# rapidsai/wholegraph

Measured on AMD Instinct MI355X. Metric: gather_GBps_out (gathered output row bytes/s, reference gather_scatter_bench convention), higher is better.
Workload: dtype f32

## Files before the change

include/wholememory/wholegraph_amd_ext.h:

```cpp
#ifndef WHOLEMEMORY_WHOLEGRAPH_AMD_EXT_H_
#define WHOLEMEMORY_WHOLEGRAPH_AMD_EXT_H_

#include <wholememory/embedding.h>
#include <wholememory/wholememory_op.h>

#ifdef __cplusplus
extern "C" {
#endif

struct wm_ext_collectives_t {
  void* ctx;
  int (*barrier)(void* ctx);
  int (*allgather_host)(void* ctx, const void* send, void* recv, size_t bytes);
  int (*alltoallv_device)(void* ctx,
                          const void* send,
                          const size_t* send_bytes,
                          const size_t* send_disp,
                          void* recv,
                          const size_t* recv_bytes,
                          const size_t* recv_disp,
                          void* stream);
};
#ifndef __cplusplus
typedef struct wm_ext_collectives_t wm_ext_collectives_t;
// ... 62 lines not shown
wholememory_error_code_t wholememory_ext_sample_append_unique(
  wholememory_tensor_t wm_csr_row_ptr_tensor, wholememory_tensor_t wm_csr_col_ptr_tensor,
  wholememory_tensor_t center_nodes_tensor, int max_sample_count, unsigned long long random_seed,
  wholememory_tensor_t output_sample_offset_tensor, void* output_unique_memory_context,
  void* output_neighbor_pos_memory_context, void* output_center_localid_memory_context, wholememory_env_func_t* p_env_fns,
  void* stream);

wholememory_error_code_t wholememory_ext_weighted_sample_append_unique(
  wholememory_tensor_t wm_csr_row_ptr_tensor, wholememory_tensor_t wm_csr_col_ptr_tensor,
  wholememory_tensor_t wm_csr_weight_ptr_tensor, wholememory_tensor_t center_nodes_tensor, int max_sample_count,
  unsigned long long random_seed, wholememory_tensor_t output_sample_offset_tensor, void* output_unique_memory_context,
  void* output_neighbor_pos_memory_context, void* output_center_localid_memory_context, wholememory_env_func_t* p_env_fns,
  void* stream);

enum wholememory_error_code_t wholememory_ext_multilayer_sample(
  wholememory_tensor_t wm_csr_row_ptr_tensor, wholememory_tensor_t wm_csr_col_ptr_tensor, wholememory_tensor_t seed_nodes_tensor,
  int hops, const int* max_sample_counts, const unsigned long long* random_seeds, void* const* sample_offsets,
  void* const* unique, int* const* neighbor_pos, int* const* center_lid, int* counts_host,
  struct wholememory_env_func_t* p_env_fns, void* stream);

enum wholememory_error_code_t wholememory_ext_multilayer_sample_weighted(
  wholememory_tensor_t wm_csr_row_ptr_tensor, wholememory_tensor_t wm_csr_col_ptr_tensor,
  wholememory_tensor_t wm_csr_weight_ptr_tensor, wholememory_tensor_t seed_nodes_tensor, int hops, const int* max_sample_counts,
  const unsigned long long* random_seeds, void* const* sample_offsets, void* const* unique, int* const* neighbor_pos,
  int* const* center_lid, int* counts_host, struct wholememory_env_func_t* p_env_fns, void* stream);

enum wholememory_error_code_t wholememory_ext_sample_append_unique_edges(
  wholememory_tensor_t wm_csr_row_ptr_tensor, wholememory_tensor_t wm_csr_col_ptr_tensor,
  wholememory_tensor_t wm_csr_weight_ptr_tensor, wholememory_tensor_t center_nodes_tensor, int max_sample_count,
  unsigned long long random_seed, wholememory_tensor_t output_sample_offset_tensor, void* output_unique_memory_context,
  void* output_neighbor_pos_memory_context, void* output_center_localid_memory_context, void* output_edge_gid_memory_context,
  struct wholememory_env_func_t* p_env_fns, void* stream);

enum wholememory_error_code_t wholememory_ext_multilayer_sample_edges(
  wholememory_tensor_t wm_csr_row_ptr_tensor, wholememory_tensor_t wm_csr_col_ptr_tensor,
  wholememory_tensor_t wm_csr_weight_ptr_tensor, wholememory_tensor_t seed_nodes_tensor, int hops, const int* max_sample_counts,
  const unsigned long long* random_seeds, void* const* sample_offsets, void* const* unique, int* const* neighbor_pos,
  int* const* center_lid, int64_t* const* edge_gid, int n_attrs, const wholememory_tensor_t* attr_tensors,
  void* const* attr_out, int* counts_host, struct wholememory_env_func_t* p_env_fns, void* stream);

int64_t wholememory_ext_edge_chain_calls(void);

enum wholememory_error_code_t wholememory_ext_set_async_completion(int on);

enum wholememory_error_code_t wholememory_ext_reload_knobs(void);

enum wholememory_error_code_t wholememory_ext_probe_memory(void* ptr, size_t bytes, int kind, int reps, float* ms_per_gib);

enum wholememory_error_code_t wholememory_ext_set_malloc_probe(const char* mode);
enum wholememory_error_code_t wholememory_ext_get_malloc_probe(char* mode, size_t capacity);
int wholememory_ext_handle_was_probed(wholememory_handle_t handle);

int64_t wholememory_ext_host_sorted_gathers(void);

int64_t wholememory_ext_split_sorts(void);

void wholememory_ext_agg_grid_stats(int64_t* launches, int64_t* truncated);

int64_t wholememory_ext_dense_fold_last(void);

int64_t wholememory_ext_distributed_gather_launches(void);

int64_t wholememory_ext_distributed_scatter_launches(void);

int64_t wholememory_ext_gradient_exchange_launches(void);

int64_t wholememory_ext_alltoallv_bytes(void);

int64_t wholememory_ext_combined_gradient_calls(void);

enum wholememory_ext_aggr_t {
  WHOLEMEMORY_EXT_AGGR_SUM  = 0,
  WHOLEMEMORY_EXT_AGGR_MEAN = 1,
};
enum wholememory_error_code_t wholememory_ext_csc_aggregate_forward(const int32_t* row_ptr,
                                                                    const int32_t* col_ind,
                                                                    int64_t n_edges,
                                                                    int64_t n_dst,
                                                                    int64_t n_src,
                                                                    const float* x,
                                                                    int64_t x_stride,
                                                                    int64_t dim,
                                                                    int aggr,
                                                                    float* out,
                                                                    int64_t out_stride,
                                                                    struct wholememory_env_func_t* p_env_fns,
                                                                    void* stream);
enum wholememory_error_code_t wholememory_ext_csc_aggregate_backward(const int32_t* row_ptr,
                                                                     const int32_t* col_ind,
                                                                     int64_t n_edges,
                                                                     int64_t n_dst,
                                                                     int64_t n_src,
                                                                     const float* grad_out,
                                                                     int64_t grad_out_stride,
                                                                     int64_t dim,
                                                                     int aggr,
                                                                     float* grad_x,
                                                                     int64_t grad_x_stride,
                                                                     struct wholememory_env_func_t* p_env_fns,
                                                                     void* stream);
int64_t wholememory_ext_csc_aggregate_chunk_edges(void);

enum wholememory_error_code_t wholememory_ext_csc_aggregate_forward_typed(const int32_t* row_ptr,
                                                                          const int32_t* col_ind,
                                                                          int64_t n_edges,
                                                                          int64_t n_dst,
// ... 450 lines not shown
```

wholegraph_amd/binding.py:

```python
import ctypes as C
import os

_HERE = os.path.dirname(os.path.abspath(__file__))
LIB_PATH = os.path.join(_HERE, "libwholegraph.so")

WHOLEMEMORY_SUCCESS = 0
NOT_SUPPORTED = 9
OUT_OF_MEMORY = 8
ERROR_NAMES = {
    0: "WHOLEMEMORY_SUCCESS", 1: "WHOLEMEMORY_UNKNOW_ERROR", 2: "WHOLEMEMORY_NOT_IMPLEMENTED",
    3: "WHOLEMEMORY_LOGIC_ERROR", 4: "WHOLEMEMORY_CUDA_ERROR", 5: "WHOLEMEMORY_COMMUNICATION_ERROR",
    6: "WHOLEMEMORY_INVALID_INPUT", 7: "WHOLEMEMORY_INVALID_VALUE", 8: "WHOLEMEMORY_OUT_OF_MEMORY",
    9: "WHOLEMEMORY_NOT_SUPPORTED", 10: "WHOLEMEMORY_SYSTEM_ERROR",
}
MT_NONE, MT_CONTINUOUS, MT_CHUNKED, MT_DISTRIBUTED, MT_HIERARCHY = range(5)
ML_NONE, ML_DEVICE, ML_HOST = range(3)
(DT_UNKNOWN, DT_FLOAT, DT_HALF, DT_DOUBLE, DT_BF16, DT_INT, DT_INT64, DT_INT16, DT_INT8, DT_COUNT) = range(10)
MA_NONE, MA_DEVICE, MA_HOST, MA_PINNED = range(4)
AGGR_SUM, AGGR_MEAN = range(2)
PNA_AGGR = {"sum": 1, "mean": 2, "min": 4, "max": 8, "std": 16}
OPT_NONE, OPT_SGD, OPT_LAZY_ADAM, OPT_RMSPROP, OPT_ADAGRAD = range(5)
AT_NONE, AT_READONLY, AT_READWRITE = range(3)
LEVEL_FATAL, LEVEL_ERROR, LEVEL_WARN, LEVEL_INFO, LEVEL_DEBUG, LEVEL_TRACE = range(6)
MAX_TENSOR_DIM = 8
# ... 161 lines not shown
    "wholememory_tensor_get_entry_partition_sizes": (_i, [_P(_sz), _vp]),
    "wholememory_tensor_get_local_entry_count": (_i, [_P(_sz), _vp]),
    "wholememory_tensor_get_local_entry_start": (_i, [_P(_sz), _vp]),
    "wholememory_tensor_get_subtensor": (_i, [_vp, _P(_i64), _P(_i64), _P(_vp)]),
    "wholememory_tensor_get_root": (_vp, [_vp]),
    "get_wholememory_tensor_count": (_i64, []),
    "get_device_prop": (_vp, [_i]),
    "wholememory_get_default_env_func": (_P(EnvFunc), []),
    "wholememory_get_cached_env_func": (_P(EnvFunc), []),
    "wholememory_drop_cached_env_func_cache": (None, []),
    "wholememory_gather": (_i, [_vp, _vp, _vp, _P(EnvFunc), _vp, _i]),
    "wholememory_scatter": (_i, [_vp, _vp, _vp, _P(EnvFunc), _vp, _i]),
    "wholememory_create_embedding_optimizer": (_i, [_P(_vp), _i]),
    "wholememory_optimizer_set_parameter": (_i, [_vp, C.c_char_p, _vp]),
    "wholememory_destroy_embedding_optimizer": (None, [_vp]),
    "wholememory_create_embedding_cache_policy": (_i, [_P(_vp), _vp, _i, _i, _i, _f]),
    "wholememory_destroy_embedding_cache_policy": (_i, [_vp]),
    "wholememory_create_embedding": (_i, [_P(_vp), _P(TensorDescription), _vp, _i, _i, _vp, _P(_sz), _i, _i]),
    "wholememory_destroy_embedding": (_i, [_vp]),
    "wholememory_embedding_get_embedding_tensor": (_vp, [_vp]),
    "wholememory_embedding_set_optimizer": (_i, [_vp, _vp]),
    "wholememory_embedding_gather": (_i, [_vp, _vp, _vp, _b, _P(EnvFunc), _i64]),
    "wholememory_embedding_gather_gradient_apply": (_i, [_vp, _vp, _vp, _b, _f, _P(EnvFunc), _i64]),
    "wholememory_embedding_get_optimizer_state_names": (_P(C.c_char_p), [_vp]),
    "wholememory_embedding_get_optimizer_state": (_vp, [_vp, C.c_char_p]),
    "wholememory_embedding_writeback_cache": (_i, [_vp, _i64]),
    "wholememory_embedding_drop_all_cache": (_i, [_vp, _i64]),
    "wholememory_env_test_op": (_i, [_vp, _vp, _vp, _vp, _vp, _i64, _P(EnvFunc), _vp]),
    "wholegraph_csr_unweighted_sample_without_replacement": (_i, [_vp, _vp, _vp, _i, _vp, _vp, _vp, _vp, C.c_ulonglong,
                                                                 _P(EnvFunc), _vp]),
    "wholegraph_csr_weighted_sample_without_replacement": (_i, [_vp, _vp, _vp, _vp, _i, _vp, _vp, _vp, _vp,
                                                               C.c_ulonglong, _P(EnvFunc), _vp]),
    "generate_random_positive_int_cpu": (_i, [_i64, _i64, _vp]),
    "generate_exponential_distribution_negative_float_cpu": (_i, [_i64, _i64, _vp]),
    "graph_append_unique": (_i, [_vp, _vp, _vp, _vp, _P(EnvFunc), _vp]),
    "csr_add_self_loop": (_i, [_vp, _vp, _vp, _vp, _vp]),
    "wholememory_create_communicator_ext": (_i, [_P(_vp), _i, _i, _P(ExtCollectives)]),
    "wholememory_ext_communicator_transport": (_i, [_vp, _P(C.c_char_p), _P(_i)]),
    "wholememory_ext_bucket_ids": (_i, [_vp, _i, _i64, _vp, _i, _vp, _vp, _vp, _P(EnvFunc), _vp]),
    "wholememory_ext_bucket_ids_folded": (_i, [_vp, _i, _i64, _vp, _i, _i, _vp, _vp, _vp, _P(EnvFunc), _vp]),
    "wholememory_ext_dedup_apply": (_i, [_vp, _i, _i64, _vp, _i64, _i64, _vp, _i64, _i64, _i64, _i, _P(_f), _f, _vp,
                                        _vp, _P(_i64), _P(EnvFunc), _vp]),
    "wholememory_ext_round_robin_map": (_i, [_vp, _vp, _i, _i64, _i64, _i, _i, _vp]),
    "wholememory_ext_embedding_cache_info": (_i, [_vp, _P(_i64), _P(_i64), _P(_i64), _P(_i64), _P(_i64)]),
    "wholememory_ext_backend_name": (C.c_char_p, []),
    "wholememory_ext_last_rows_kernel": (C.c_char_p, []),
    "wholememory_ext_sample_append_unique": (C.c_int, [C.c_void_p, C.c_void_p, C.c_void_p, C.c_int, C.c_ulonglong, C.c_void_p,
                                                      C.c_void_p, C.c_void_p, C.c_void_p, C.c_void_p, C.c_void_p]),
    "wholememory_ext_weighted_sample_append_unique": (_i, [_vp, _vp, _vp, _vp, _i, C.c_ulonglong, _vp, _vp, _vp, _vp, _vp, _vp]),
    "wholememory_ext_set_async_completion": (_i, [_i]),
    "wholememory_ext_reload_knobs": (_i, []),
    "wholememory_ext_probe_memory": (_i, [_vp, C.c_size_t, _i, _i, _P(_f)]),
    "wholememory_ext_host_sorted_gathers": (_i64, []),
    "wholememory_ext_split_sorts": (_i64, []),
    "wholememory_ext_agg_grid_stats": (None, [_P(_i64), _P(_i64)]),
    "wholememory_ext_dense_fold_last": (_i64, []),
    "wholememory_ext_distributed_gather_launches": (_i64, []),
    "wholememory_ext_distributed_scatter_launches": (_i64, []),
    "wholememory_ext_gradient_exchange_launches": (_i64, []),
    "wholememory_ext_alltoallv_bytes": (_i64, []),
    "wholememory_ext_combined_gradient_calls": (_i64, []),
    "wholememory_ext_set_malloc_probe": (_i, [C.c_char_p]),
    "wholememory_ext_get_malloc_probe": (_i, [C.c_char_p, C.c_size_t]),
    "wholememory_ext_handle_was_probed": (_i, [_vp]),
    "wholememory_ext_multilayer_sample": (_i, [_vp, _vp, _vp, _i, _vp, _vp, _vp, _vp, _vp, _vp, _vp, _vp, _vp]),
    "wholememory_ext_multilayer_sample_weighted": (_i, [_vp, _vp, _vp, _vp, _i, _vp, _vp, _vp, _vp, _vp, _vp, _vp, _vp, _vp]),
    "wholememory_ext_sample_append_unique_edges": (_i, [_vp, _vp, _vp, _vp, _i, C.c_ulonglong, _vp, _vp, _vp, _vp, _vp, _vp, _vp]),
    "wholememory_ext_multilayer_sample_edges": (_i, [_vp, _vp, _vp, _vp, _i, _vp, _vp, _vp, _vp, _vp, _vp, _vp, _i, _vp, _vp, _vp,
                                                    _vp, _vp]),
    "wholememory_ext_edge_chain_calls": (_i64, []),
    "wholememory_ext_csr_random_walk": (_i, [_vp, _vp, _vp, _vp, _i, C.c_ulonglong, _vp, _vp, _vp]),
    "wholememory_ext_csr_node2vec_walk": (_i, [_vp, _vp, _vp, _vp, _i, C.c_float, C.c_float, _i, C.c_ulonglong, _vp, _vp, _vp]),
    "wholememory_ext_csr_negative_sample": (_i, [_vp, _vp, _vp, _i, _i, _i, _i, _i, C.c_ulonglong, _vp, _vp]),
    "wholememory_ext_csr_induced_subgraph": (_i, [_vp, _vp, _vp, _vp, _vp, _vp, _P(EnvFunc), _vp]),
    "wholememory_ext_csc_aggregate_forward": (_i, [_vp, _vp, _i64, _i64, _i64, _vp, _i64, _i64, _i, _vp, _i64, _P(EnvFunc),
                                                  _vp]),
    "wholememory_ext_csc_aggregate_backward": (_i, [_vp, _vp, _i64, _i64, _i64, _vp, _i64, _i64, _i, _vp, _i64, _P(EnvFunc),
                                                   _vp]),
    "wholememory_ext_csc_aggregate_chunk_edges": (_i64, []),
    "wholememory_ext_csc_aggregate_forward_typed": (_i, [_vp, _vp, _i64, _i64, _i64, _vp, _i64, _i64, _i, _vp, _i64, _i,
                                                        _P(EnvFunc), _vp]),
    "wholememory_ext_csc_aggregate_backward_typed": (_i, [_vp, _vp, _i64, _i64, _i64, _vp, _i64, _i64, _i, _vp, _i64, _i,
                                                         _P(EnvFunc), _vp]),
    "wholememory_ext_csc_aggregate_weighted_forward": (_i, [_vp, _vp, _vp, _i64, _i64, _i64, _vp, _i64, _i64, _i, _vp, _i64,
                                                           _P(EnvFunc), _vp]),
    "wholememory_ext_csc_gather_aggregate_forward": (_i, [_vp, _vp, _i, _vp, _vp, _i64, _i64, _i64, _i, _vp, _i64, _P(EnvFunc),
                                                         _vp]),
    "wholememory_ext_gather_aggregate_calls": (_i64, []),
    "wholememory_ext_csc_aggregate_weighted_backward": (_i, [_vp, _vp, _i64, _i64, _i64, _vp, _i64, _vp, _vp, _i64, _i64, _i,
                                                            _vp, _i64, _vp, _P(EnvFunc), _vp]),
    "wholememory_ext_csc_gat_forward": (_i, [_vp, _vp, _i64, _i64, _i64, _vp, _i64, _vp, _i64, _i64, C.c_float, _i, _vp,
                                            _i64, _vp, _vp, _P(EnvFunc), _vp]),
    "wholememory_ext_csc_gat_backward": (_i, [_vp, _vp, _i64, _i64, _i64, _vp, _i64, _vp, _i64, _i64, C.c_float, _i, _vp,
                                             _vp, _vp, _i64, _vp, _i64, _vp, _P(EnvFunc), _vp]),
    "wholememory_ext_csc_gat_node_chunk": (_i64, []),
    "wholememory_ext_csc_gat_edge_forward": (_i, [_vp, _vp, _i64, _i64, _i64, _vp, _i64, _vp, _vp, _i64, _i64, _i64,
                                                 C.c_float, _i, _vp, _i64, _vp, _vp, _vp, _P(EnvFunc), _vp]),
    "wholememory_ext_csc_gat_edge_backward": (_i, [_vp, _vp, _i64, _i64, _i64, _vp, _i64, _vp, _vp, _i64, _i64, _i64,
                                                  C.c_float, _i, _vp, _vp, _vp, _vp, _i64, _vp, _i64, _vp, _vp, _i64,
                                                  _P(EnvFunc), _vp]),
    "wholememory_ext_csc_gatv2_forward": (_i, [_vp, _vp, _i64, _i64, _i64, _vp, _i64, _vp, _i64, _vp, _i64, _i64,
                                              C.c_float, _i, _vp, _i64, _vp, _P(EnvFunc), _vp]),
    "wholememory_ext_csc_gatv2_backward": (_i, [_vp, _vp, _i64, _i64, _i64, _vp, _i64, _vp, _i64, _vp, _i64, _i64,
                                               C.c_float, _i, _vp, _vp, _i64, _vp, _i64, _vp, _i64, _vp, _P(EnvFunc),
                                               _vp]),
    "wholememory_ext_csc_mha_simple_forward": (_i, [_vp, _vp, _i64, _i64, _i64, _vp, _i64, _vp, _i64, _vp, _i64, _i64, _i64,
# ... 72 lines not shown
```

wholegraph_amd/csrc/embedding_cache.cpp:

```cpp
#include "embedding_cache.hpp"

#include <algorithm>
#include <cstring>

namespace wm {

row_cache::~row_cache()
{
  const auto* bk = backend();
  if (args.slot_of) bk->free_device(args.slot_of);
  if (args.count) bk->free_device(args.count);
  if (args.row_of) bk->free_device(args.row_of);
  if (args.dirty) bk->free_device(args.dirty);
  if (args.data) bk->free_device(args.data);
  if (args.data2) bk->free_device(args.data2);
  if (counters_dev) bk->free_device(counters_dev);
}

wholememory_error_code_t create_row_cache(row_cache** out, const wholememory_embedding_cache_policy_* policy,
                                          wholememory_tensor_t raw, wholememory_comm_t embedding_comm)
{
  const auto* bk = backend();
  if (bk->cache_update == nullptr) return WHOLEMEMORY_NOT_SUPPORTED;
  auto* desc = wholememory_tensor_get_tensor_description(raw);
  auto h     = wholememory_tensor_get_memory_handle(raw);
  std::unique_ptr<row_cache> c(new row_cache());
  c->same_comm = policy->cache_comm == embedding_comm;
  c->writable  = policy->access_type == WHOLEMEMORY_AT_READWRITE;
  c->dtype     = desc->dtype;
  c->row_elems = desc->strides[0];
  c->raw       = raw;
  const size_t es = wholememory_dtype_get_element_size(desc->dtype);
  auto& a         = c->args;
  a.row_bytes     = c->row_elems * static_cast<int64_t>(es);
  if (a.row_bytes % 16 != 0) return WHOLEMEMORY_LOGIC_ERROR;
  a.raw_row_stride_bytes = a.row_bytes;
  a.raw_row_offset_bytes = desc->storage_offset * static_cast<int64_t>(es);
  if (c->same_comm) {
    std::vector<size_t> off = entry_offsets_of(h, static_cast<size_t>(a.row_bytes));
    a.cover_start           = static_cast<int64_t>(off[embedding_comm->world_rank]);
    a.cover_rows            = static_cast<int64_t>(off[embedding_comm->world_rank + 1]) - a.cover_start;
    a.raw_gref              = local_shard_gref(h);
  } else {
    a.cover_start = 0;
    a.cover_rows  = desc->sizes[0];
    if (wholememory_get_memory_type(h) == WHOLEMEMORY_MT_DISTRIBUTED && embedding_comm->world_size > 1) {
      c->raw_addressable = false;
      a.raw_gref         = wholememory_create_continuous_global_reference(nullptr);
    } else {
      WHOLEMEMORY_RETURN_ON_FAIL(tensor_mapped_gref(raw, &a.raw_gref));
    }
  }
  if (a.cover_rows >= (INT64_C(1) << 31)) return WHOLEMEMORY_NOT_SUPPORTED;
  int64_t slots = static_cast<int64_t>(static_cast<double>(a.cover_rows) * policy->cache_ratio);
  slots         = std::min(a.cover_rows + 63, std::max<int64_t>(slots, a.cover_rows > 0 ? 64 : 0));
  a.n_sets      = (slots + 63) / 64;
  a.set_cover   = a.n_sets > 0 ? (a.cover_rows + a.n_sets - 1) / a.n_sets : 0;
  const int64_t n_slots = a.n_sets * 64;
  auto dev_alloc = [&](void** p, size_t bytes) { WM_BK(bk->malloc_device(p, std::max<size_t>(bytes, 16))); };
  dev_alloc(reinterpret_cast<void**>(&a.slot_of), sizeof(int32_t) * a.cover_rows);
  dev_alloc(reinterpret_cast<void**>(&a.count), sizeof(int32_t) * a.cover_rows);
  dev_alloc(reinterpret_cast<void**>(&a.row_of), sizeof(int64_t) * n_slots);
  dev_alloc(reinterpret_cast<void**>(&a.dirty), n_slots);
  dev_alloc(reinterpret_cast<void**>(&a.data), static_cast<size_t>(n_slots) * a.row_bytes);
  dev_alloc(reinterpret_cast<void**>(&c->counters_dev), 32);
  WM_BK(bk->memset_async(a.slot_of, 0xff, sizeof(int32_t) * a.cover_rows, nullptr));
  WM_BK(bk->memset_async(a.count, 0, sizeof(int32_t) * a.cover_rows, nullptr));
  WM_BK(bk->memset_async(a.row_of, 0xff, sizeof(int64_t) * n_slots, nullptr));
  WM_BK(bk->memset_async(a.dirty, 0, n_slots, nullptr));
  WM_BK(bk->memset_async(c->counters_dev, 0, 32, nullptr));
  WM_BK(bk->stream_sync(nullptr));
  *out = c.release();
  return WHOLEMEMORY_SUCCESS;
}

wholememory_error_code_t row_cache_update(row_cache* c, const void* ids, wholememory_dtype_t index_dtype, int64_t n,
                                          int64_t key_upper_bound, wholememory_env_func_t* env, void* stream)
{
  const auto* bk = backend();
  if (n == 0 || c->args.n_sets == 0) return WHOLEMEMORY_SUCCESS;
  if (n >= (INT64_C(1) << 31)) return WHOLEMEMORY_INVALID_INPUT;
  sorted_ids s(env);
  int rc = s.run(ids, index_dtype, n, key_upper_bound, 0, stream);
  if (rc != 0) return rc == -1 ? WHOLEMEMORY_INVALID_INPUT : WHOLEMEMORY_CUDA_ERROR;
  rc = bk->cache_update(&c->args, s.unique, index_dtype, s.starts, s.n_unique_dev, n, nullptr, nullptr, nullptr, stream);
  if (rc != 0) return rc == -1 ? WHOLEMEMORY_INVALID_INPUT : WHOLEMEMORY_CUDA_ERROR;
  WM_BK(bk->stream_sync(stream));
  return WHOLEMEMORY_SUCCESS;
}

wholememory_error_code_t row_cache_plan(row_cache* c, const void* ids, wholememory_dtype_t index_dtype, int64_t n, int64_t key_upper_bound,
                                        wholememory_env_func_t* env, void* stream, temp_mem* rows_mem, temp_mem* slots_mem,
                                        int64_t* n_fill)
{
  const auto* bk = backend();
  *n_fill        = 0;
  auto* fill_rows  = static_cast<int64_t*>(rows_mem->device(n, WHOLEMEMORY_DT_INT64));
  auto* fill_slots = static_cast<int64_t*>(slots_mem->device(n, WHOLEMEMORY_DT_INT64));
  if (n == 0 || c->args.n_sets == 0) return WHOLEMEMORY_SUCCESS;
  if (n >= (INT64_C(1) << 31) || c->writable) return WHOLEMEMORY_INVALID_INPUT;
  sorted_ids s(env);
  temp_mem count(env), host_n(env);
  auto* d_count = static_cast<int*>(count.device(1, WHOLEMEMORY_DT_INT));
  WM_BK(bk->memset_async(d_count, 0, sizeof(int), stream));
  int rc = s.run(ids, index_dtype, n, key_upper_bound, 0, stream);
  if (rc != 0) return rc == -1 ? WHOLEMEMORY_INVALID_INPUT : WHOLEMEMORY_CUDA_ERROR;
  rc = bk->cache_update(&c->args, s.unique, index_dtype, s.starts, s.n_unique_dev, n, fill_rows, fill_slots, d_count, stream);
  if (rc != 0) return rc == -1 ? WHOLEMEMORY_INVALID_INPUT : WHOLEMEMORY_CUDA_ERROR;
  auto* h = static_cast<int*>(host_n.pinned(1, WHOLEMEMORY_DT_INT));
  WM_BK(bk->memcpy_async(h, d_count, sizeof(int), stream));
  WM_BK(bk->stream_sync(stream));
  *n_fill = *h;
  return WHOLEMEMORY_SUCCESS;
}

wholememory_error_code_t row_cache_install(row_cache* c, const void* rows_data, const int64_t* slots, int64_t n_fill,
                                           void* stream)
{
  const auto* bk = backend();
  if (n_fill == 0) return WHOLEMEMORY_SUCCESS;
  wm_rows_args a{};
  a.gref          = wholememory_create_continuous_global_reference(c->args.data);
  a.table_dtype   = c->dtype;
  a.dim           = c->row_elems;
  a.table_stride  = c->row_elems;
  a.indices       = slots;
  a.index_dtype   = WHOLEMEMORY_DT_INT64;
  a.n             = n_fill;
  a.plain         = const_cast<void*>(rows_data);
  a.plain_dtype   = c->dtype;
  a.plain_stride  = c->row_elems;
  a.max_blocks    = -1;
  WM_BK(bk->scatter_rows(&a, stream));
  return WHOLEMEMORY_SUCCESS;
}

wholememory_error_code_t row_cache_split(row_cache* c, const void* ids, wholememory_dtype_t index_dtype, int64_t n,
                                         int64_t* cache_idx, void* raw_idx, void* stream)
{
  int rc = backend()->cache_split(&c->args, ids, index_dtype, n, cache_idx, raw_idx, c->counters_dev, stream);
  if (rc != 0) return rc == -1 ? WHOLEMEMORY_INVALID_INPUT : WHOLEMEMORY_CUDA_ERROR;
  c->lookups += n;
  return WHOLEMEMORY_SUCCESS;
}

wholememory_error_code_t row_cache_gather(row_cache* c, const wm_rows_args& a, wholememory_env_func_t* env, void* stream)
{
  const auto* bk = backend();
  if (a.n == 0) return WHOLEMEMORY_SUCCESS;
  temp_mem cache_idx_mem(env), raw_idx_mem(env);
  auto* cache_idx = static_cast<int64_t*>(cache_idx_mem.device(a.n, WHOLEMEMORY_DT_INT64));
  void* raw_idx   = raw_idx_mem.device(a.n, a.index_dtype);
  WHOLEMEMORY_RETURN_ON_FAIL(row_cache_split(c, a.indices, a.index_dtype, a.n, cache_idx, raw_idx, stream));
  wm_rows_args hit        = a;
  hit.gref                = wholememory_create_continuous_global_reference(c->args.data);
  hit.table_stride        = c->row_elems;
  hit.table_storage_offset = 0;
  hit.indices             = cache_idx;
  hit.index_dtype         = WHOLEMEMORY_DT_INT64;
  WM_BK(bk->gather_rows(&hit, stream));
  wm_rows_args miss = a;
  miss.indices      = raw_idx;
  WM_BK(bk->gather_rows(&miss, stream));
  WM_BK(bk->stream_sync(stream));
  return WHOLEMEMORY_SUCCESS;
}

wholememory_error_code_t row_cache_attach_states(row_cache* c, wholememory_tensor_t state_local)
{
  const auto* bk = backend();
  if (!c->same_comm || !c->writable || c->args.data2 != nullptr) return WHOLEMEMORY_INVALID_INPUT;
  WHOLEMEMORY_RETURN_ON_FAIL(row_cache_writeback(c, true, nullptr));
  auto* d = wholememory_tensor_get_tensor_description(state_local);
  if (d->dtype != WHOLEMEMORY_DT_FLOAT || d->dim != 2) return WHOLEMEMORY_INVALID_INPUT;
  auto& a                 = c->args;
  a.row_bytes2            = d->strides[0] * static_cast<int64_t>(sizeof(float));
  a.raw2_row_stride_bytes = a.row_bytes2;
  if (a.row_bytes2 % 16 != 0) return WHOLEMEMORY_LOGIC_ERROR;
  char* local = static_cast<char*>(wholememory_tensor_get_data_pointer(state_local));
  a.raw2_gref = wholememory_create_continuous_global_reference(local - a.cover_start * a.row_bytes2);
  void* p     = nullptr;
  WM_BK(bk->malloc_device(&p, std::max<size_t>(static_cast<size_t>(a.n_sets) * 64 * a.row_bytes2, 16)));
  a.data2 = static_cast<char*>(p);
  return WHOLEMEMORY_SUCCESS;
}

wholememory_error_code_t row_cache_writeback(row_cache* c, bool drop, void* stream)
{
  const auto* bk = backend();
  int rc         = bk->cache_writeback(&c->args, drop ? 1 : 0, stream);
  if (rc != 0) return WHOLEMEMORY_CUDA_ERROR;
  return bk->stream_sync(stream) == 0 ? WHOLEMEMORY_SUCCESS : WHOLEMEMORY_CUDA_ERROR;
}

wholememory_error_code_t row_cache_info(row_cache* c, int64_t* slots, int64_t* occupied, int64_t* dirty, int64_t* hits,
                                        int64_t* lookups, void* stream)
{
  const auto* bk = backend();
  if (bk->cache_info(&c->args, c->counters_dev + 1, stream) != 0) return WHOLEMEMORY_CUDA_ERROR;
  unsigned long long h[3] = {0, 0, 0};
  WM_BK(bk->memcpy_async(h, c->counters_dev, sizeof(h), stream));
  WM_BK(bk->stream_sync(stream));
  if (slots) *slots = c->args.n_sets * 64;
  if (occupied) *occupied = static_cast<int64_t>(h[1]);
  if (dirty) *dirty = static_cast<int64_t>(h[2]);
  if (hits) *hits = static_cast<int64_t>(h[0]);
  if (lookups) *lookups = c->lookups;
  return WHOLEMEMORY_SUCCESS;
}

}
```

wholegraph_amd/csrc/embedding_cache.hpp:

```cpp
#pragma once

#include <wholememory/embedding.h>

#include "backend.hpp"
#include "ops_internal.hpp"

struct wholememory_embedding_cache_policy_ {
  wholememory_comm_t cache_comm;
  wholememory_memory_type_t cache_memory_type;
  wholememory_memory_location_t cache_memory_location;
  wholememory_access_type_t access_type;
  float cache_ratio;
};

namespace wm {

struct row_cache {
  wm_cache_args args{};
  bool same_comm = false;
  bool writable  = false;
  bool raw_addressable = true;
  wholememory_tensor_t raw = nullptr;
  wholememory_dtype_t dtype = WHOLEMEMORY_DT_UNKNOWN;
  int64_t row_elems         = 0;
  unsigned long long* counters_dev = nullptr;
  int64_t lookups                  = 0;
  ~row_cache();
};

wholememory_error_code_t create_row_cache(row_cache** out, const wholememory_embedding_cache_policy_* policy,
                                          wholememory_tensor_t raw, wholememory_comm_t embedding_comm);

wholememory_error_code_t row_cache_update(row_cache* c, const void* ids, wholememory_dtype_t index_dtype, int64_t n,
                                          int64_t key_upper_bound, wholememory_env_func_t* env, void* stream);

wholememory_error_code_t row_cache_gather(row_cache* c, const wm_rows_args& a, wholememory_env_func_t* env, void* stream);

wholememory_error_code_t row_cache_plan(row_cache* c, const void* ids, wholememory_dtype_t index_dtype, int64_t n,
                                        int64_t key_upper_bound, wholememory_env_func_t* env, void* stream, temp_mem* rows_mem, temp_mem* slots_mem,
                                        int64_t* n_fill);
wholememory_error_code_t row_cache_install(row_cache* c, const void* rows_data, const int64_t* slots, int64_t n_fill,
                                           void* stream);
wholememory_error_code_t row_cache_split(row_cache* c, const void* ids, wholememory_dtype_t index_dtype, int64_t n,
                                         int64_t* cache_idx, void* raw_idx, void* stream);

wholememory_error_code_t row_cache_attach_states(row_cache* c, wholememory_tensor_t state_local);

wholememory_error_code_t row_cache_writeback(row_cache* c, bool drop, void* stream);
wholememory_error_code_t row_cache_info(row_cache* c, int64_t* slots, int64_t* occupied, int64_t* dirty, int64_t* hits,
                                        int64_t* lookups, void* stream);

}
```

wholegraph_amd/csrc/kernels/cache.hip:

```cpp
#include <hip/hip_runtime.h>
#include <stdint.h>

#include <algorithm>

#include "../backend.hpp"

namespace wm {
namespace {

constexpr int kBlock = 256;

struct raw_view {
  char* base;
  char* const* rank_ptrs;
  const size_t* rank_offsets;
  size_t chunk_stride;
  int world_size;
  int same_chunk;
  int64_t row_stride_bytes;
  int64_t row_offset_bytes;
};

struct raw2_view {
  char* base;
// ... 29 lines not shown
  size_t start;
  if (v.same_chunk) {
    rank  = static_cast<int>(off / v.chunk_stride);
    start = static_cast<size_t>(rank) * v.chunk_stride;
  } else {
    rank = 0;
    for (int r = 1; r < v.world_size; r++)
      if (off >= v.rank_offsets[r]) rank = r;
    start = v.rank_offsets[rank];
  }
  return v.rank_ptrs[rank] + (off - start);
}

__device__ __forceinline__ void wave_copy_row(char* dst, const char* src, int row_bytes, int lane)
{
  typedef uint32_t u32x4 __attribute__((ext_vector_type(4)));
  for (int o = lane * 16; o < row_bytes; o += 64 * 16) *reinterpret_cast<u32x4*>(dst + o) = *reinterpret_cast<const u32x4*>(src + o);
}

struct cache_dev {
  int32_t* slot_of;
  int32_t* count;
  int64_t* row_of;
  uint8_t* dirty;
  char* data;
  int64_t cover_start, cover_rows, n_sets, set_cover;
  int row_bytes;
  char* data2;
  int row_bytes2;
};

inline cache_dev make_dev(const wm_cache_args& c)
{
  return cache_dev{c.slot_of, c.count, c.row_of, c.dirty, c.data, c.cover_start, c.cover_rows, c.n_sets, c.set_cover,
                   static_cast<int>(c.row_bytes), c.data2, static_cast<int>(c.row_bytes2)};
}

template <typename IdxT>
__global__ void cache_count_kernel(cache_dev c, const IdxT* unique_rows, const int32_t* run_starts, const int64_t* n_unique)
{
  const int64_t u = static_cast<int64_t>(blockIdx.x) * blockDim.x + threadIdx.x;
  if (u >= *n_unique) return;
  const int64_t r = static_cast<int64_t>(unique_rows[u]) - c.cover_start;
  if (r < 0 || r >= c.cover_rows) return;
  c.count[r] += run_starts[u + 1] - run_starts[u];
}

struct fill_list {
  int64_t* rows;
  int64_t* slots;
  int* count;
};

template <typename IdxT>
__global__ __launch_bounds__(kBlock) void cache_update_kernel(cache_dev c, raw_view raw, raw2_view raw2,
                                                              const IdxT* unique_rows, const int64_t* n_unique_p,
                                                              fill_list fill)
{
  const int lane    = threadIdx.x & 63;
  const int64_t set = (static_cast<int64_t>(blockIdx.x) * kBlock + threadIdx.x) >> 6;
  if (set >= c.n_sets) return;
  const int64_t nu  = *n_unique_p;
  const int64_t lo_row = c.cover_start + set * c.set_cover;
  const int64_t hi_row = min(c.cover_start + c.cover_rows, lo_row + c.set_cover);
  auto lower = [&](int64_t key) {
    int64_t a = 0, b = nu;
    while (a < b) {
      const int64_t m = (a + b) >> 1;
      const IdxT v    = unique_rows[m];
      if (v >= 0 && static_cast<int64_t>(v) < key)
        a = m + 1;
      else
        b = m;
    }
    return a;
  };
  const int64_t first = lower(lo_row), last = lower(hi_row);
  if (first >= last) return;
  const int64_t slot  = set * 64 + lane;
  int64_t my_row      = c.row_of[slot];
  int32_t my_cnt      = my_row >= 0 ? c.count[my_row] : -1;
  for (int64_t j = first; j < last; j++) {
    const int64_t g = static_cast<int64_t>(unique_rows[j]);
    const int64_t r = g - c.cover_start;
    if (c.slot_of[r] >= 0) continue;
    const int32_t cand = c.count[r];
    uint64_t key = (static_cast<uint64_t>(static_cast<uint32_t>(my_cnt + 1)) << 8) | static_cast<uint32_t>(lane);
    for (int off = 32; off > 0; off >>= 1) {
      const uint64_t o = __shfl_xor(key, off, 64);
      key              = o < key ? o : key;
    }
    const int victim      = static_cast<int>(key & 0xff);
    const int32_t min_cnt = static_cast<int32_t>(key >> 8) - 1;
    if (cand <= min_cnt) continue;
    const int64_t vslot = set * 64 + victim;
    char* line          = c.data + vslot * c.row_bytes;
    const int64_t old   = __shfl(my_row, victim, 64);
    if (old >= 0) {
      if (fill.rows == nullptr && c.dirty[vslot]) {
        wave_copy_row(raw_row(raw, c.cover_start + old), line, c.row_bytes, lane);
        if (c.data2 != nullptr)
          wave_copy_row(raw2.base + (c.cover_start + old) * raw2.row_stride_bytes, c.data2 + vslot * c.row_bytes2, c.row_bytes2, lane);
      }
      if (lane == 0) c.slot_of[old] = -1;
    }
    if (fill.rows == nullptr) {
      wave_copy_row(line, raw_row(raw, g), c.row_bytes, lane);
      if (c.data2 != nullptr)
        wave_copy_row(c.data2 + vslot * c.row_bytes2, raw2.base + g * raw2.row_stride_bytes, c.row_bytes2, lane);
    } else if (lane == 0) {
      const int k   = atomicAdd(fill.count, 1);
      fill.rows[k]  = g;
      fill.slots[k] = vslot;
    }
    if (lane == 0) {
      c.slot_of[r]    = static_cast<int32_t>(vslot);
      c.row_of[vslot] = r;
      c.dirty[vslot]  = 0;
    }
    if (lane == victim) {
      my_row = r;
      my_cnt = cand;
    }
    __builtin_amdgcn_fence(__ATOMIC_RELEASE, "agent");
  }
}

template <typename IdxT>
__global__ __launch_bounds__(kBlock) void cache_split_kernel(cache_dev c, const IdxT* ids, int64_t n, int64_t* cache_idx,
                                                             IdxT* raw_idx, unsigned long long* hits)
{
  __shared__ unsigned int block_hits;
  if (threadIdx.x == 0) block_hits = 0;
  __syncthreads();
  unsigned int wave_hits = 0;
  for (int64_t base = static_cast<int64_t>(blockIdx.x) * kBlock; base < n; base += static_cast<int64_t>(gridDim.x) * kBlock) {
    const int64_t i = base + threadIdx.x;
    bool hit        = false;
    if (i < n) {
      const IdxT id   = ids[i];
      const int64_t r = static_cast<int64_t>(id) - c.cover_start;
      int32_t slot    = -1;
      if (id >= 0 && r >= 0 && r < c.cover_rows) slot = c.slot_of[r];
      hit          = slot >= 0;
      cache_idx[i] = slot;
      raw_idx[i]   = hit ? static_cast<IdxT>(-1) : id;
    }
    wave_hits += static_cast<unsigned int>(__popcll(__ballot(hit)));
  }
  if (hits != nullptr) {
    if ((threadIdx.x & 63) == 0 && wave_hits) atomicAdd(&block_hits, wave_hits);
    __syncthreads();
    if (threadIdx.x == 0 && block_hits) atomicAdd(hits, static_cast<unsigned long long>(block_hits));
  }
}

__global__ __launch_bounds__(kBlock) void cache_writeback_kernel(cache_dev c, raw_view raw, raw2_view raw2, int drop)
{
  const int lane     = threadIdx.x & 63;
  const int64_t slot = (static_cast<int64_t>(blockIdx.x) * kBlock + threadIdx.x) >> 6;
  if (slot >= c.n_sets * 64) return;
  const int64_t r = c.row_of[slot];
  if (r < 0) return;
  if (c.dirty[slot]) {
    wave_copy_row(raw_row(raw, c.cover_start + r), c.data + slot * c.row_bytes, c.row_bytes, lane);
    if (c.data2 != nullptr)
      wave_copy_row(raw2.base + (c.cover_start + r) * raw2.row_stride_bytes, c.data2 + slot * c.row_bytes2, c.row_bytes2, lane);
  }
  if (lane == 0) {
    c.dirty[slot] = 0;
    if (drop) {
      c.slot_of[r]   = -1;
      c.row_of[slot] = -1;
    }
  }
}

// ... 88 lines not shown
```

wholegraph_amd/csrc/ops.cpp:

```cpp
#include "knobs.hpp"
#include "ops_internal.hpp"
#include "embedding_cache.hpp"

#include <algorithm>
#include <atomic>
#include <cstdlib>
#include <cstring>

namespace wm {

temp_mem::temp_mem(wholememory_env_func_t* env) : env_(env)
{
  WM_CHECK(env != nullptr, "p_env_fns must not be null");
  env_->temporary_fns.create_memory_context_fn(&ctx_, env_->temporary_fns.global_context);
}
temp_mem::~temp_mem()
{
  if (ptr_ != nullptr) env_->temporary_fns.free_fn(ctx_, env_->temporary_fns.global_context);
  env_->temporary_fns.destroy_memory_context_fn(ctx_, env_->temporary_fns.global_context);
}
void* temp_mem::alloc(int64_t elt_count, wholememory_dtype_t dtype, wholememory_memory_allocation_type_t type)
{
  WM_CHECK(ptr_ == nullptr, "temp_mem slot reused");
  wholememory_tensor_description_t d;
// ... 675 lines not shown
  temp_mem fetched(env), relay_rows(env), back_rows(env);
  char* fetched_buf = static_cast<char*>(fetched.device(dim * n_fetch, d.plain.dtype));
  op_descs db       = d;
  db.indices_ptr    = fetch_ids;
  db.indices        = wholememory_create_array_desc(n_fetch, 0, d.indices.dtype);
  db.plain_ptr      = fetched_buf;
  int64_t fsz[2]    = {n_fetch, dim};
  db.plain          = wholememory_create_matrix_desc(fsz, dim, 0, d.plain.dtype);
  WHOLEMEMORY_RETURN_ON_FAIL(gather_distributed_rows(handle, db, env, stream, gather_sms, nullptr, false, &rail));

  char* send_buf = fetched_buf;
  WM_DEBUG("HIERARCHY gather: rank %d (local %d of %d, node %d of %d) asked %ld ids, relays %ld, fetches %ld distinct",
           comm->world_rank, local_comm->world_rank, L, cross_comm->world_rank, X, static_cast<long>(n),
           static_cast<long>(n_relay), static_cast<long>(n_fetch));
  if (dedup) {
    send_buf       = static_cast<char*>(relay_rows.device(dim * n_relay, d.plain.dtype));
    int64_t rsz[2] = {n_relay, dim};
    auto relay_desc = wholememory_create_matrix_desc(rsz, dim, 0, d.plain.dtype);
    wm_rows_args ea{};
    fill_rows_args(&ea, wholememory_create_continuous_global_reference(fetched_buf), db.plain, inv, WHOLEMEMORY_DT_INT64,
                   n_relay, send_buf, relay_desc, gather_sms);
    WM_BK(bk->gather_rows(&ea, stream));
  }

  const size_t row_bytes = static_cast<size_t>(dim) * oes;
  char* back_buf = static_cast<char*>(back_rows.device(dim * xa.total_valid, d.plain.dtype));
  exchange_segments(local_comm, send_buf, xa.recv_counts, xa.recv_offsets, back_buf, xa.send_counts, xa.bucket_offsets,
                    row_bytes, stream);
  if (xa.total_valid > 0) {
    int64_t bsz[2] = {xa.total_valid, dim};
    auto back_desc = wholememory_create_matrix_desc(bsz, dim, 0, d.plain.dtype);
    wm_rows_args ra{};
    fill_rows_args(&ra, wholememory_create_continuous_global_reference(d.plain_ptr), d.plain, xa.raw_indices,
                   WHOLEMEMORY_DT_INT64, xa.total_valid, back_buf, back_desc, -1);
    WM_BK(bk->scatter_rows(&ra, stream));
  }
  WM_BK(bk->stream_sync(stream));
  return WHOLEMEMORY_SUCCESS;
}

}

wholememory_error_code_t gather_cached(wholememory_tensor_t table, wholememory_tensor_t indices_tensor,
                                       wholememory_tensor_t output_tensor, wholememory_env_func_t* env, void* stream,
                                       int gather_sms, row_cache* cache, bool adjust_cache)
{
  op_descs d;
  WHOLEMEMORY_RETURN_ON_FAIL(check_args(table, indices_tensor, output_tensor, "output", &d));
  auto handle = wholememory_tensor_get_memory_handle(table);
  if (cache->same_comm)
    return gather_distributed_rows(handle, d, env, stream, gather_sms, cache, adjust_cache);
  if (cache->raw_addressable) {
    if (adjust_cache)
      WHOLEMEMORY_RETURN_ON_FAIL(row_cache_update(cache, d.indices_ptr, d.indices.dtype, d.indices.size, d.table.sizes[0], env, stream));
    wm_rows_args a{};
    fill_rows_args(&a, cache->args.raw_gref, d.table, d.indices_ptr, d.indices.dtype, d.indices.size, d.plain_ptr, d.plain,
                   gather_sms);
    return row_cache_gather(cache, a, env, stream);
  }
  const auto* bk     = backend();
  const int64_t n    = d.indices.size;
  const int64_t dim  = d.table.sizes[1];
  if (adjust_cache) {
    temp_mem rows_mem(env), slots_mem(env), staging(env);
    int64_t n_fill = 0;
    WHOLEMEMORY_RETURN_ON_FAIL(row_cache_plan(cache, d.indices_ptr, d.indices.dtype, n, d.table.sizes[0], env, stream, &rows_mem, &slots_mem, &n_fill));
    char* rows_data = static_cast<char*>(staging.device(n_fill * cache->row_elems, d.table.dtype));
    op_descs df     = d;
    df.indices_ptr  = rows_mem.get();
    df.indices      = wholememory_create_array_desc(n_fill, 0, WHOLEMEMORY_DT_INT64);
    df.plain_ptr    = rows_data;
    int64_t fsz[2]  = {n_fill, dim};
    df.plain        = wholememory_create_matrix_desc(fsz, cache->row_elems, 0, d.table.dtype);
    WHOLEMEMORY_RETURN_ON_FAIL(gather_distributed_rows(handle, df, env, stream, gather_sms));
    WHOLEMEMORY_RETURN_ON_FAIL(row_cache_install(cache, rows_data, static_cast<const int64_t*>(slots_mem.get()), n_fill, stream));
    WM_BK(bk->stream_sync(stream));
  }
  temp_mem cache_idx_mem(env), raw_idx_mem(env);
  auto* cache_idx = static_cast<int64_t*>(cache_idx_mem.device(n, WHOLEMEMORY_DT_INT64));
  void* raw_idx   = raw_idx_mem.device(n, d.indices.dtype);
  WHOLEMEMORY_RETURN_ON_FAIL(row_cache_split(cache, d.indices_ptr, d.indices.dtype, n, cache_idx, raw_idx, stream));
  if (n > 0) {
    wm_rows_args hit{};
    fill_rows_args(&hit, wholememory_create_continuous_global_reference(cache->args.data), d.table, cache_idx,
                   WHOLEMEMORY_DT_INT64, n, d.plain_ptr, d.plain, gather_sms);
    hit.table_stride         = cache->row_elems;
    hit.table_storage_offset = 0;
    WM_BK(bk->gather_rows(&hit, stream));
  }
  op_descs dm    = d;
  dm.indices_ptr = raw_idx;
  dm.indices.storage_offset = 0;
  WHOLEMEMORY_RETURN_ON_FAIL(gather_distributed(handle, dm, env, stream, gather_sms));
  WM_BK(bk->stream_sync(stream));
  return WHOLEMEMORY_SUCCESS;
}

namespace {

wholememory_error_code_t scatter_distributed(wholememory_handle_t handle, const op_descs& d,
                                             wholememory_env_func_t* env, void* stream, int scatter_sms)
{
  const auto* bk = backend();
  if (d.table.storage_offset < 0 || d.table.storage_offset + d.table.sizes[1] > d.table.stride)
    return WHOLEMEMORY_INVALID_INPUT;
  wholememory_comm_t comm;
  WHOLEMEMORY_RETURN_ON_FAIL(wholememory_get_communicator(&comm, handle));
  const size_t tes    = wholememory_dtype_get_element_size(d.table.dtype);
  const size_t pes    = wholememory_dtype_get_element_size(d.plain.dtype);
  const size_t ies    = wholememory_dtype_get_element_size(d.indices.dtype);
  const int64_t dim   = d.table.sizes[1];
// ... 237 lines not shown
```

Before: 2926.

## Batch cache update per wave, search set bounds wave-wide, and drop gather syncs

Rewrites the cache update kernel. Each wave now finds its set's index range with a 64-way ballot search instead of a serial binary search. It then scans candidate rows in chunks, resolves all victim replacements in registers first, and only afterwards does one batched writeback and fill copy across all changed slots. It also lets the cached gather and update paths return without a stream sync when async completion is enabled. An env knob to force the plan route and a planned-rows counter are added as well. This cuts serialized per-candidate copies, fences and host syncs, but the reordering changes eviction semantics: a row evicted and reinstalled within one call is only written back at the end.

```diff
diff --git a/include/wholememory/wholegraph_amd_ext.h b/include/wholememory/wholegraph_amd_ext.h
--- a/include/wholememory/wholegraph_amd_ext.h
+++ b/include/wholememory/wholegraph_amd_ext.h
@@ -138,6 +138,8 @@
 int wholememory_ext_handle_was_probed(wholememory_handle_t handle);
 
 int64_t wholememory_ext_host_sorted_gathers(void);
+
+int64_t wholememory_ext_cache_planned_rows(void);
 
 int64_t wholememory_ext_split_sorts(void);
 
diff --git a/wholegraph_amd/binding.py b/wholegraph_amd/binding.py
--- a/wholegraph_amd/binding.py
+++ b/wholegraph_amd/binding.py
@@ -237,6 +237,7 @@
     "wholememory_ext_reload_knobs": (_i, []),
     "wholememory_ext_probe_memory": (_i, [_vp, C.c_size_t, _i, _i, _P(_f)]),
     "wholememory_ext_host_sorted_gathers": (_i64, []),
+    "wholememory_ext_cache_planned_rows": (_i64, []),
     "wholememory_ext_split_sorts": (_i64, []),
     "wholememory_ext_agg_grid_stats": (None, [_P(_i64), _P(_i64)]),
     "wholememory_ext_dense_fold_last": (_i64, []),
diff --git a/wholegraph_amd/csrc/embedding_cache.cpp b/wholegraph_amd/csrc/embedding_cache.cpp
--- a/wholegraph_amd/csrc/embedding_cache.cpp
+++ b/wholegraph_amd/csrc/embedding_cache.cpp
@@ -1,9 +1,22 @@
 #include "embedding_cache.hpp"
 
 #include <algorithm>
+#include <atomic>
 #include <cstring>
 
+#include "knobs.hpp"
+
 namespace wm {
+
+namespace {
+std::atomic<int64_t> g_cache_planned_rows{0};
+
+bool plan_route_forced()
+{
+  const char* e = WM_KNOB("WM_CACHE_PLAN");
+  return e != nullptr && e[0] == '1';
+}
+}
 
 row_cache::~row_cache()
 {
@@ -44,7 +57,7 @@
   } else {
     a.cover_start = 0;
     a.cover_rows  = desc->sizes[0];
-    if (wholememory_get_memory_type(h) == WHOLEMEMORY_MT_DISTRIBUTED && embedding_comm->world_size > 1) {
+    if (wholememory_get_memory_type(h) == WHOLEMEMORY_MT_DISTRIBUTED && (embedding_comm->world_size > 1 || plan_route_forced())) {
       c->raw_addressable = false;
       a.raw_gref         = wholememory_create_continuous_global_reference(nullptr);
     } else {
@@ -75,7 +88,8 @@
 }
 
 wholememory_error_code_t row_cache_update(row_cache* c, const void* ids, wholememory_dtype_t index_dtype, int64_t n,
-                                          int64_t key_upper_bound, wholememory_env_func_t* env, void* stream)
+                                          int64_t key_upper_bound, wholememory_env_func_t* env, void* stream,
+                                          bool may_return_queued)
 {
   const auto* bk = backend();
   if (n == 0 || c->args.n_sets == 0) return WHOLEMEMORY_SUCCESS;
@@ -85,7 +99,7 @@
   if (rc != 0) return rc == -1 ? WHOLEMEMORY_INVALID_INPUT : WHOLEMEMORY_CUDA_ERROR;
   rc = bk->cache_update(&c->args, s.unique, index_dtype, s.starts, s.n_unique_dev, n, nullptr, nullptr, nullptr, stream);
   if (rc != 0) return rc == -1 ? WHOLEMEMORY_INVALID_INPUT : WHOLEMEMORY_CUDA_ERROR;
-  WM_BK(bk->stream_sync(stream));
+  if (!may_return_queued || !async_completion_enabled() || debug_sync_enabled()) WM_BK(bk->stream_sync(stream));
   return WHOLEMEMORY_SUCCESS;
 }
 
@@ -111,6 +125,7 @@
   WM_BK(bk->memcpy_async(h, d_count, sizeof(int), stream));
   WM_BK(bk->stream_sync(stream));
   *n_fill = *h;
+  g_cache_planned_rows.fetch_add(*h, std::memory_order_relaxed);
   return WHOLEMEMORY_SUCCESS;
 }
 
@@ -144,7 +159,8 @@
   return WHOLEMEMORY_SUCCESS;
 }
 
-wholememory_error_code_t row_cache_gather(row_cache* c, const wm_rows_args& a, wholememory_env_func_t* env, void* stream)
+wholememory_error_code_t row_cache_gather(row_cache* c, const wm_rows_args& a, wholememory_env_func_t* env, void* stream,
+                                          bool may_return_queued)
 {
   const auto* bk = backend();
   if (a.n == 0) return WHOLEMEMORY_SUCCESS;
@@ -162,7 +178,7 @@
   wm_rows_args miss = a;
   miss.indices      = raw_idx;
   WM_BK(bk->gather_rows(&miss, stream));
-  WM_BK(bk->stream_sync(stream));
+  if (!may_return_queued || !async_completion_enabled() || debug_sync_enabled()) WM_BK(bk->stream_sync(stream));
   return WHOLEMEMORY_SUCCESS;
 }
 
@@ -210,3 +226,5 @@
 }
 
 }
+
+extern "C" int64_t wholememory_ext_cache_planned_rows(void) { return wm::g_cache_planned_rows.load(std::memory_order_relaxed); }
diff --git a/wholegraph_amd/csrc/embedding_cache.hpp b/wholegraph_amd/csrc/embedding_cache.hpp
--- a/wholegraph_amd/csrc/embedding_cache.hpp
+++ b/wholegraph_amd/csrc/embedding_cache.hpp
@@ -32,9 +32,11 @@
                                           wholememory_tensor_t raw, wholememory_comm_t embedding_comm);
 
 wholememory_error_code_t row_cache_update(row_cache* c, const void* ids, wholememory_dtype_t index_dtype, int64_t n,
-                                          int64_t key_upper_bound, wholememory_env_func_t* env, void* stream);
+                                          int64_t key_upper_bound, wholememory_env_func_t* env, void* stream,
+                                          bool may_return_queued = false);
 
-wholememory_error_code_t row_cache_gather(row_cache* c, const wm_rows_args& a, wholememory_env_func_t* env, void* stream);
+wholememory_error_code_t row_cache_gather(row_cache* c, const wm_rows_args& a, wholememory_env_func_t* env, void* stream,
+                                          bool may_return_queued = false);
 
 wholememory_error_code_t row_cache_plan(row_cache* c, const void* ids, wholememory_dtype_t index_dtype, int64_t n,
                                         int64_t key_upper_bound, wholememory_env_func_t* env, void* stream, temp_mem* rows_mem, temp_mem* slots_mem,
diff --git a/wholegraph_amd/csrc/kernels/cache.hip b/wholegraph_amd/csrc/kernels/cache.hip
--- a/wholegraph_amd/csrc/kernels/cache.hip
+++ b/wholegraph_amd/csrc/kernels/cache.hip
@@ -105,6 +105,44 @@
   int* count;
 };
 
+__device__ __forceinline__ int nth_set_bit(uint64_t m, int k)
+{
+  int pos = 0;
+  for (int w = 32; w > 0; w >>= 1) {
+    const int below = __popcll((m >> pos) & ((1ull << w) - 1));
+    if (k >= below) {
+      k -= below;
+      pos += w;
+    }
+  }
+  return pos;
+}
+
+__device__ __forceinline__ void wave_copy_rows(uint64_t m, char* my_dst, const char* my_src, int bytes, int lane)
+{
+  typedef uint32_t u32x4 __attribute__((ext_vector_type(4)));
+  const int n      = __popcll(m);
+  const int pieces = bytes >> 4;
+  const auto d64   = reinterpret_cast<unsigned long long>(my_dst);
+  const auto s64   = reinterpret_cast<unsigned long long>(my_src);
+  if (pieces <= 32) {
+    const int per_pass = 64 / pieces, sub = lane / pieces, off = (lane - sub * pieces) * 16;
+    for (int base = 0; base < n; base += per_pass) {
+      const int k       = base + sub;
+      const bool active = sub < per_pass && k < n;
+      const int l       = nth_set_bit(m, active ? k : 0);
+      char* dst         = reinterpret_cast<char*>(__shfl(d64, l, 64));
+      const char* src   = reinterpret_cast<const char*>(__shfl(s64, l, 64));
+      if (active) *reinterpret_cast<u32x4*>(dst + off) = *reinterpret_cast<const u32x4*>(src + off);
+    }
+  } else {
+    for (uint64_t rest = m; rest != 0; rest &= rest - 1) {
+      const int l = __builtin_amdgcn_readfirstlane(__ffsll(static_cast<unsigned long long>(rest)) - 1);
+      wave_copy_row(reinterpret_cast<char*>(__shfl(d64, l, 64)), reinterpret_cast<const char*>(__shfl(s64, l, 64)), bytes, lane);
+    }
+  }
+}
+
 template <typename IdxT>
 __global__ __launch_bounds__(kBlock) void cache_update_kernel(cache_dev c, raw_view raw, raw2_view raw2,
                                                               const IdxT* unique_rows, const int64_t* n_unique_p,
@@ -116,66 +154,110 @@
   const int64_t nu  = *n_unique_p;
   const int64_t lo_row = c.cover_start + set * c.set_cover;
   const int64_t hi_row = min(c.cover_start + c.cover_rows, lo_row + c.set_cover);
-  auto lower = [&](int64_t key) {
-    int64_t a = 0, b = nu;
-    while (a < b) {
-      const int64_t m = (a + b) >> 1;
-      const IdxT v    = unique_rows[m];
-      if (v >= 0 && static_cast<int64_t>(v) < key)
-        a = m + 1;
-      else
-        b = m;
-    }
-    return a;
+  int64_t first = 0;
+  for (int64_t end = nu; first < end;) {
+    const int64_t len  = end - first;
+    const int64_t step = len > 64 ? len >> 6 : 1;
+    const int64_t p    = first + (lane + 1) * step - 1;
+    bool below         = false;
+    if (p < end) {
+      const IdxT v = unique_rows[p];
+      below        = v >= 0 && static_cast<int64_t>(v) < lo_row;
+    }
+    const int k = __popcll(__ballot(below));
+    if (len <= 64) {
+      first += k;
+      break;
+    }
+    if (k < 64) end = first + (k + 1) * step - 1;
+    first += k * step;
+  }
+  auto chunk_row = [&](int64_t from) {
+    const int64_t j = from + lane;
+    int32_t r       = -1;
+    if (j < nu) {
+      const IdxT v = unique_rows[j];
+      if (v >= 0 && static_cast<int64_t>(v) < hi_row) r = static_cast<int32_t>(static_cast<int64_t>(v) - c.cover_start);
+    }
+    return r;
   };
-  const int64_t first = lower(lo_row), last = lower(hi_row);
-  if (first >= last) return;
-  const int64_t slot  = set * 64 + lane;
-  int64_t my_row      = c.row_of[slot];
-  int32_t my_cnt      = my_row >= 0 ? c.count[my_row] : -1;
-  for (int64_t j = first; j < last; j++) {
-    const int64_t g = static_cast<int64_t>(unique_rows[j]);
-    const int64_t r = g - c.cover_start;
-    if (c.slot_of[r] >= 0) continue;
-    const int32_t cand = c.count[r];
+  int32_t r = chunk_row(first);
+  if (__ballot(r >= 0) == 0) return;
+  const int64_t slot     = set * 64 + lane;
+  const int32_t orig_row = static_cast<int32_t>(c.row_of[slot]);
+  const bool was_dirty   = c.dirty[slot] != 0;
+  int32_t my_row         = orig_row;
+  int32_t my_cnt         = orig_row >= 0 ? c.count[orig_row] : -1;
+  int victim;
+  int32_t min_cnt;
+  auto pick_victim = [&]() {
     uint64_t key = (static_cast<uint64_t>(static_cast<uint32_t>(my_cnt + 1)) << 8) | static_cast<uint32_t>(lane);
     for (int off = 32; off > 0; off >>= 1) {
       const uint64_t o = __shfl_xor(key, off, 64);
       key              = o < key ? o : key;
     }
-    const int victim      = static_cast<int>(key & 0xff);
-    const int32_t min_cnt = static_cast<int32_t>(key >> 8) - 1;
-    if (cand <= min_cnt) continue;
-    const int64_t vslot = set * 64 + victim;
-    char* line          = c.data + vslot * c.row_bytes;
-    const int64_t old   = __shfl(my_row, victim, 64);
-    if (old >= 0) {
-      if (fill.rows == nullptr && c.dirty[vslot]) {
-        wave_copy_row(raw_row(raw, c.cover_start + old), line, c.row_bytes, lane);
-        if (c.data2 != nullptr)
-          wave_copy_row(raw2.base + (c.cover_start + old) * raw2.row_stride_bytes, c.data2 + vslot * c.row_bytes2, c.row_bytes2, lane);
+    victim  = static_cast<int>(key & 0xff);
+    min_cnt = static_cast<int32_t>(key >> 8) - 1;
+  };
+  bool picked = false;
+  for (int64_t from = first;; from += 64) {
+    const bool in_set   = r >= 0;
+    const int n_rows    = __popcll(__ballot(in_set));
+    const int32_t so    = in_set ? c.slot_of[r] : 0;
+    const int32_t cnt   = in_set ? c.count[r] : 0;
+    if (!picked) {
+      pick_victim();
+      picked = true;
+    }
+    uint64_t cands = __ballot(in_set && so < 0 && cnt > min_cnt);
+    while (cands != 0) {
+      const int src = __builtin_amdgcn_readfirstlane(__ffsll(static_cast<unsigned long long>(cands)) - 1);
+      const int32_t cand_row = __builtin_amdgcn_readlane(r, src);
+      const int32_t cand_cnt = __builtin_amdgcn_readlane(cnt, src);
+      if (lane == victim) {
+        my_row = cand_row;
+        my_cnt = cand_cnt;
       }
-      if (lane == 0) c.slot_of[old] = -1;
-    }
-    if (fill.rows == nullptr) {
-      wave_copy_row(line, raw_row(raw, g), c.row_bytes, lane);
-      if (c.data2 != nullptr)
-        wave_copy_row(c.data2 + vslot * c.row_bytes2, raw2.base + g * raw2.row_stride_bytes, c.row_bytes2, lane);
-    } else if (lane == 0) {
+      pick_victim();
+      cands &= ~((2ull << src) - 1);
+      cands &= __ballot(cnt > min_cnt);
+    }
+    if (n_rows < 64) break;
+    r = chunk_row(from + 64);
+    if (__ballot(r >= 0) == 0) break;
+  }
+
+  const bool changed     = my_row != orig_row;
+  const uint64_t changes = __ballot(changed);
+  if (changes == 0) return;
+  char* line       = c.data + slot * c.row_bytes;
+  char* line2      = c.data2 != nullptr ? c.data2 + slot * c.row_bytes2 : nullptr;
+  const bool plan  = fill.rows != nullptr;
+  if (!plan) {
+    const bool back       = changed && orig_row >= 0 && was_dirty;
+    const uint64_t backs  = __ballot(back);
+    if (backs != 0) {
+      const int64_t g_old = c.cover_start + orig_row;
+      wave_copy_rows(backs, back ? raw_row(raw, g_old) : nullptr, line, c.row_bytes, lane);
+      if (c.data2 != nullptr) wave_copy_rows(backs, raw2.base + g_old * raw2.row_stride_bytes, line2, c.row_bytes2, lane);
+      __builtin_amdgcn_wave_barrier();
+    }
+  }
+  const int64_t g_new = c.cover_start + my_row;
+  if (changed) {
+    if (orig_row >= 0) c.slot_of[orig_row] = -1;
+    c.slot_of[my_row] = static_cast<int32_t>(slot);
+    c.row_of[slot]    = my_row;
+    c.dirty[slot]     = 0;
+    if (plan) {
       const int k   = atomicAdd(fill.count, 1);
-      fill.rows[k]  = g;
-      fill.slots[k] = vslot;
-    }
-    if (lane == 0) {
-      c.slot_of[r]    = static_cast<int32_t>(vslot);
-      c.row_of[vslot] = r;
-      c.dirty[vslot]  = 0;
-    }
-    if (lane == victim) {
-      my_row = r;
-      my_cnt = cand;
-    }
-    __builtin_amdgcn_fence(__ATOMIC_RELEASE, "agent");
+      fill.rows[k]  = g_new;
+      fill.slots[k] = slot;
+    }
+  }
+  if (!plan) {
+    wave_copy_rows(changes, line, changed ? raw_row(raw, g_new) : nullptr, c.row_bytes, lane);
+    if (c.data2 != nullptr) wave_copy_rows(changes, line2, raw2.base + g_new * raw2.row_stride_bytes, c.row_bytes2, lane);
   }
 }
 
diff --git a/wholegraph_amd/csrc/ops.cpp b/wholegraph_amd/csrc/ops.cpp
--- a/wholegraph_amd/csrc/ops.cpp
+++ b/wholegraph_amd/csrc/ops.cpp
@@ -751,11 +751,11 @@
     return gather_distributed_rows(handle, d, env, stream, gather_sms, cache, adjust_cache);
   if (cache->raw_addressable) {
     if (adjust_cache)
-      WHOLEMEMORY_RETURN_ON_FAIL(row_cache_update(cache, d.indices_ptr, d.indices.dtype, d.indices.size, d.table.sizes[0], env, stream));
+      WHOLEMEMORY_RETURN_ON_FAIL(row_cache_update(cache, d.indices_ptr, d.indices.dtype, d.indices.size, d.table.sizes[0], env, stream, true));
     wm_rows_args a{};
     fill_rows_args(&a, cache->args.raw_gref, d.table, d.indices_ptr, d.indices.dtype, d.indices.size, d.plain_ptr, d.plain,
                    gather_sms);
-    return row_cache_gather(cache, a, env, stream);
+    return row_cache_gather(cache, a, env, stream, true);
   }
   const auto* bk     = backend();
   const int64_t n    = d.indices.size;
```

Measured after the change: 2926. Within noise of the previous version (-0.0%).
